# grantjr1842/index-tts

Measured on AMD Instinct MI355X. Metric: synthesised audio seconds per second (IndexTTS-2 infer_v2 hot path), whole job, higher is better.
Workload: dtype f32 (greedy decode + its prefill: exact fp32 MFMA; fp32 accumulate and fp32 activations everywhere) + split-bf16 (fp32 operands as hi+lo bf16, 3 bf16 MFMAs per product) GEMMs, DiT attention and convolutions in s2mel, the latent pass and the vocoder; GPT linear weights STORED as bf16 (rounded once at

## Files before the change

include/idxtts.h:

```cpp
#ifndef IDXTTS_H
#define IDXTTS_H

#include <stddef.h>
#include <stdint.h>

#ifdef __cplusplus
extern "C" {
#endif

typedef struct idxtts_ctx idxtts_ctx;

#define IDXTTS_DTYPE_F32 0
#define IDXTTS_DTYPE_F16 1
#define IDXTTS_DTYPE_BF16 2

int idxtts_version(void);
const char* idxtts_last_error(void);

int idxtts_aa_act_fwd(void* out, const void* in, const float* up_filter, const float* down_filter,
                      const float* log_alpha, const float* log_beta, int B, int C, int T, int dtype,
                      void* stream);

typedef struct idxtts_conv1d idxtts_conv1d;
int idxtts_conv1d_create(const float* weight, const float* bias , int Cout, int Cin, int K,
// ... 39 lines not shown
int idxtts_set_gemm_mode(int mode);
int idxtts_get_gemm_mode(void);
int idxtts_set_acoustic_bf16(int on);
int idxtts_get_acoustic_bf16(void);
int idxtts_set_decode_geometry(int narrow);
int idxtts_get_decode_geometry(void);
int idxtts_set_decode_plane_rows(int min_rows);
int idxtts_get_decode_plane_rows(void);
typedef struct idxtts_gemv_fx_plan {
  int mt, ntw, single, r4, narrow, kw, cps, ksb;
} idxtts_gemv_fx_plan;
int idxtts_gemv_fx_plan_query(int N, int K, int rows, int format, int with_slab, int narrow, idxtts_gemv_fx_plan* out);
int idxtts_gemv_pl_plan_query(int N, int K, int rows, int* ct, int* kparts, int* has_kernel);
int idxtts_s2mel_set_overlap(int on);
int idxtts_s2mel_get_overlap(void);
int idxtts_linear_destroy(idxtts_linear* lin);
int idxtts_release_stream(void* stream);
int idxtts_attention_fwd(const float* q, const float* k, const float* v, float* o, long q_batch_stride, int q_token_stride,
                         long kv_batch_stride, int kv_token_stride, long o_batch_stride, int o_token_stride, int B, int H,
                         int Sq, int Sk, int causal, const int* kstart, const int* kend, float scale, void* stream);
int idxtts_attention_bf16x3_fwd(const float* q, const float* k, const float* v, float* o, long q_batch_stride, int q_token_stride,
                         long kv_batch_stride, int kv_token_stride, long o_batch_stride, int o_token_stride, int B, int H,
                         int Sq, int Sk, int causal, const int* kstart, const int* kend, float scale, void* stream);
int idxtts_attention_bf16_fwd(const float* q, const float* k, const float* v, float* o, long q_batch_stride, int q_token_stride,
                         long kv_batch_stride, int kv_token_stride, long o_batch_stride, int o_token_stride, int B, int H,
                         int Sq, int Sk, int causal, const int* kstart, const int* kend, float scale, void* stream);
int idxtts_attention_relkey_fwd(const float* q, const float* k, const float* v, float* o, long batch_stride, int token_stride,
                                long o_batch_stride, int o_token_stride, int B, int H, int S, const int* kend, float scale,
                                const float* rel_key, int rel_left, int rel_right, int split_bf16, void* stream);
int idxtts_layernorm_fwd(const float* x, float* y, const float* gamma, const float* beta, int M, int d, float eps, void* stream);
// ... 222 lines not shown
```

index-tts_amd/csrc/attention.h:

```cpp
#pragma once
#include "common.h"

namespace idxtts {

struct AttnArgs {
  const float* q = nullptr; const float* k = nullptr; const float* v = nullptr; float* o = nullptr;
  long q_bs = 0, k_bs = 0, v_bs = 0, o_bs = 0;
  int q_ts = 0, k_ts = 0, v_ts = 0, o_ts = 0;
  int B = 0, H = 0, Sq = 0, Sk = 0, head_dim = 64;
  int causal = 0;
  const int* kstart = nullptr;
  const int* kend = nullptr;
  float scale = 0.125f;
  void* o_planes = nullptr;
  int split_bf16 = 0;
  const float* rel_key = nullptr; int rel_left = 0, rel_right = 0;
};

int flash_attn_forward(const AttnArgs& a, hipStream_t stream);

struct AttnPlanesArgs {
  const void* planes = nullptr;
  int Mrows = 0, ncols = 0;
  int q_col = 0, k_col = 0, v_col = 0;
  int T = 0;
// ... 13 lines not shown
```

index-tts_amd/csrc/attention.hip:

```cpp
#include <algorithm>

#include "attention.h"
#include "prof.h"

namespace idxtts {

__device__ __forceinline__ float xor32_max(float v) {
  const auto r = __builtin_amdgcn_permlane32_swap(__float_as_uint(v), __float_as_uint(v), false, false);
  return fmaxf(__uint_as_float(r[0]), __uint_as_float(r[1]));
}
__device__ __forceinline__ float xor32_sum(float v) {
  const auto r = __builtin_amdgcn_permlane32_swap(__float_as_uint(v), __float_as_uint(v), false, false);
  return __uint_as_float(r[0]) + __uint_as_float(r[1]);
}

constexpr int KROW = 68;
constexpr float NEG_BIG = -1e30f;
constexpr int REL_MAX = 96;
constexpr int REL_ROW = 97;
constexpr int REL_LDS = 4 * 32 * REL_ROW * (int)sizeof(float);
constexpr int STAGE_FLOATS = 4 * 32 * 65;

__device__ __forceinline__ int acc_key(int r, int h, int key0 = 0) { return key0 + (r & 3) + 8 * (r >> 2) + 4 * h; }

// ... 8 lines not shown
  w.h = w.lane >> 5; w.j = w.lane & 31;
  w.q0 = qblk * 128 + w.wave * 32;
  w.qi = w.q0 + w.j;
  return w;
}

struct KeyRange {
  int kstart, kend, k_lo, ntiles;
  __device__ __forceinline__ bool sees(int key, int qi, int causal) const { return key >= kstart && key < kend && (!causal || key <= qi); }
};
__device__ __forceinline__ KeyRange visible_keys(const AttnArgs& p, int b, int qblk) {
  KeyRange k;
  k.kstart = p.kstart ? p.kstart[b] : 0;
  k.kend = p.kend ? min(p.kend[b], p.Sk) : p.Sk;
  int k_hi = k.kend;
  if (p.causal) k_hi = min(k_hi, qblk * 128 + 128);
  k.k_lo = k.kstart & ~31;
  k.ntiles = k_hi > k.k_lo ? (k_hi - k.k_lo + 31) >> 5 : 0;
  return k;
}

__device__ __forceinline__ void load_kv(const AttnArgs& p, const float* kb, const float* vb, int key0, int tid, f32x4 (&kr)[2], f32x4 (&vr)[2]) {
#pragma unroll
  for (int l = 0; l < 2; ++l) {
    const int idx = tid + 256 * l;
    const int row = idx >> 4, c4 = idx & 15;
    const int key = key0 + row;
    f32x4 a = {0.f, 0.f, 0.f, 0.f}, c = {0.f, 0.f, 0.f, 0.f};
    if (key < p.Sk) {
      a = *reinterpret_cast<const f32x4*>(kb + (size_t)key * p.k_ts + c4 * 4);
      c = *reinterpret_cast<const f32x4*>(vb + (size_t)key * p.v_ts + c4 * 4);
// ... 118 lines not shown
  extern __shared__ float rel_dyn[];
  float* const tbl_row = rel_dyn + (w.wave * 32 + w.j) * REL_ROW;
  if (p.rel_key)
    build_rel_table(p, w, tbl_row, [&](int row, int c4, f32x4 a) { store_k(0, row, c4, a); }, [&] { return qk_f32(Ks[0], qf, w); });

  if (keys.ntiles > 0) {
    load_kv(p, kb, vb, keys.k_lo, w.tid, kr, vr);
    store_kv(0);
  }
  __syncthreads();
  for (int tile = 0; tile < keys.ntiles; ++tile) {
    const bool has_next = tile + 1 < keys.ntiles;
    const int key0 = keys.k_lo + tile * 32;
    if (has_next) load_kv(p, kb, vb, key0 + 32, w.tid, kr, vr);
    const float* vt = Vs[tile & 1];
    const bool wave_active = !(p.causal && key0 > w.q0 + 31) && w.q0 < p.Sq;
    if (wave_active) {
      f32x16 s = qk_f32(Ks[tile & 1], qf, w);
      if (p.rel_key) add_rel_term(s, tbl_row, key0, w, p.rel_left, p.rel_right);
      float mx = NEG_BIG;
#pragma unroll
      for (int r = 0; r < 16; ++r) {
        s[r] = keys.sees(acc_key(r, w.h, key0), w.qi, p.causal) ? s[r] : NEG_BIG;
        mx = fmaxf(mx, s[r]);
      }
      mx = xor32_max(mx);
      const float m_new = fmaxf(m_run, mx);
      const float alpha = expf(m_run - m_new);
      float psum = 0.0f;
#pragma unroll
      for (int r = 0; r < 16; ++r) {
        const float pv = s[r] <= -1e29f ? 0.0f : expf(s[r] - m_new);
        s[r] = pv;
        psum += pv;
      }
      l_run = l_run * alpha + psum;
      m_run = m_new;
#pragma unroll
// ... 150 lines not shown

  extern __shared__ float rel_dyn[];
  float* const tbl_row = rel_dyn + (w.wave * 32 + w.j) * REL_ROW;
  if (p.rel_key) build_rel_table(p, w, tbl_row, [&](int row, int c4, f32x4 a) { store_k(smem, row, c4, a); }, [&] { return qk(smem); });

  if (keys.ntiles > 0) {
    load_kv(p, kb, vb, keys.k_lo, w.tid, kr, vr);
    store_kv(0);
  }
  __syncthreads();
  for (int tile = 0; tile < keys.ntiles; ++tile) {
    const bool has_next = tile + 1 < keys.ntiles;
    const int key0 = keys.k_lo + tile * 32;
    if (has_next) load_kv(p, kb, vb, key0 + 32, w.tid, kr, vr);
    const char* tb = smem + (tile & 1) * ABUF;
    const bool wave_active = !(p.causal && key0 > w.q0 + 31) && w.q0 < p.Sq;
    if (wave_active) {
      f32x16 s = qk(tb);
      if (p.rel_key) add_rel_term(s, tbl_row, key0, w, p.rel_left, p.rel_right);
      const bool need_mask = key0 < keys.kstart || key0 + 32 > keys.kend || (p.causal && key0 + 31 > w.q0);
      if (need_mask) {
#pragma unroll
        for (int r = 0; r < 16; ++r) s[r] = keys.sees(acc_key(r, w.h, key0), w.qi, p.causal) ? s[r] : NEG_BIG;
      }
      online_softmax_log2<NP == 1>(s, o, m_run, l_run, p.scale * 1.4426950408889634f, need_mask);
      bf16x8 ph[2], pl[2];
      split_p(s, ph, pl);
#pragma unroll
      for (int t2 = 0; t2 < 2; ++t2)
#pragma unroll
        for (int t = 0; t < 2; ++t) {
          const char* va = tb + v_off + 16 * t2 * VB16 + 64 * t;
          typedef __attribute__((address_space(3))) bf16x4 lds_bf16x4;
          const bf16x4 h0 = __builtin_amdgcn_ds_read_tr16_b64_v4bf16((lds_bf16x4*)(va));
          const bf16x4 h1 = __builtin_amdgcn_ds_read_tr16_b64_v4bf16((lds_bf16x4*)(va + 8 * VB16));
          const bf16x8 vh = __builtin_shufflevector(h0, h1, 0, 1, 2, 3, 4, 5, 6, 7);
          bf16x8 vl = vh;
          if constexpr (NP == 3) {
// ... 155 lines not shown
  const double flops = 4.0 * a.B * a.H * (double)a.Sq * a.T * 64;
  const double bytes = 4.0 * a.B * a.H * 64.0 * (2.0 * a.Sq + 2.0 * a.T);
  static const int cat = prof_register("flash_attn_planes_kernel");
  ProfScope prof(cat, stream, flops, bytes);
  IDX_CHECK(a.split_bf16 == 1 || a.split_bf16 == 2, "split_bf16: 1 (three MFMAs per product) or 2 (one)");
  if (a.split_bf16 == 2) hipLaunchKernelGGL(flash_attn_planes_kernel<1>, grid, dim3(256), 0, stream, k);
  else hipLaunchKernelGGL(flash_attn_planes_kernel<3>, grid, dim3(256), 0, stream, k);
  IDX_LAUNCH_CHECK();
  return 0;
}

int flash_attn_forward(const AttnArgs& a, hipStream_t stream) {
  if (a.B == 0 || a.H == 0 || a.Sq == 0) return 0;
  IDX_CHECK(a.q && a.k && a.v && (a.o || (a.o_planes && a.split_bf16)), "null pointer");
  IDX_CHECK(a.head_dim == 64, "head_dim must be 64");
  IDX_CHECK((a.q_ts & 3) == 0 && (a.k_ts & 3) == 0 && (a.v_ts & 3) == 0 && (a.q_bs & 3) == 0 && (a.k_bs & 3) == 0 && (a.v_bs & 3) == 0,
            "q/k/v strides must be multiples of 4 floats");
  dim3 grid(cdiv(a.Sq, 128), a.H, a.B);
  const double flops = 4.0 * a.B * a.H * (double)a.Sq * a.Sk * 64 * (a.causal ? 0.5 : 1.0);
  const double bytes = 4.0 * a.B * a.H * 64.0 * (2.0 * a.Sq + 2.0 * a.Sk);
  static const int cat_x3 = prof_register("flash_attn_bf16x3_kernel"), cat_f32 = prof_register("flash_attn_f32_kernel");
  ProfScope prof(a.split_bf16 ? cat_x3 : cat_f32, stream, flops, bytes);
  size_t dyn = 0;
  if (a.rel_key) {
    IDX_CHECK(a.rel_left >= 0 && a.rel_right >= 0 && a.rel_left + a.rel_right + 1 <= REL_MAX && !a.causal && a.Sq == a.Sk && !a.kstart,
              "relative_key: non-causal self-attention, at most 96 distances");
    IDX_CHECK((reinterpret_cast<uintptr_t>(a.rel_key) & 15) == 0, "rel_key must be 16-byte aligned");
    dyn = REL_LDS;
    static DynLdsLimit lds_limit;
    IDX_CHECK(a.split_bf16 != 2, "relative_key has no single-product form");
// ... 12 lines not shown
```

index-tts_amd/csrc/capi.hip:

```cpp
#include <cstring>
#include <new>

#include "../../include/idxtts.h"
#include "bigvgan.h"
#include "cond.h"
#include "semantic.h"
#include "codec.h"
#include "audio.h"
#include "campplus.h"
#include "conv1d.h"
#include "ctx.h"
#include "fbank.h"
#include "gpt.h"
#include "model_util.h"
#include "s2mel.h"

namespace idxtts {

static thread_local std::string g_last_error;

void set_error(const std::string& msg) { g_last_error = msg; }
int fail(const char* file, int line, const std::string& msg) {
  const char* base = std::strrchr(file, '/');
  g_last_error = std::string(base ? base + 1 : file) + ":" + std::to_string(line) + ": " + msg;
// ... 851 lines not shown
  API_BEGIN
  IDX_CHECK(ct && kparts && has_kernel && N > 0 && K > 0 && rows > 0 && rows <= 64, "N, K > 0, 1..64 rows");
  gemv_pl_plan(N, K, rows, ct, kparts);
  *has_kernel = gemv_pl_can_run(N, K, rows) ? 1 : 0;
  return 0;
  API_END
}

int idxtts_s2mel_set_overlap(int on) {
  set_s2mel_overlap(on);
  return 0;
}

int idxtts_s2mel_get_overlap(void) { return get_s2mel_overlap(); }

}
```

index-tts_amd/csrc/gpt.h:

```cpp
#pragma once
#include <atomic>
#include <functional>
#include <map>
#include <mutex>
#include <vector>

#include "../../include/idxtts.h"
#include "attention.h"
#include "beam.h"
#include "ctx.h"
#include "decode.h"
#include "gemm.h"
#include "gemv16.h"
#include "gemv_pl.h"
#include "norm.h"
#include "prof.h"

namespace idxtts {

struct BeamBuffers {
  float *proc, *beam_scores;
  int *next_tok, *beam_idx, *seq, *hyp_len, *hyp_slot, *hyp_seq, *hyp_n, *done;
  double *hyp_score, *hyp_worst;
  size_t bytes;
// ... 31 lines not shown
  struct GenScope { GPTModel* m; explicit GenScope(GPTModel* mm) : m(mm) { m->generating.fetch_add(1); } ~GenScope() { m->generating.fetch_sub(1); } };
  size_t kv_layer_bytes(int B, int Smax) const { return (size_t)B * cfg.heads * Smax * 64 * (kv_fmt == 2 ? 1 : kv_fmt ? 2 : 4); }
  size_t kv_layer_scales(int B, int Smax) const { return kv_fmt == 2 ? (size_t)B * cfg.heads * Smax : 0; }
  hipStream_t own_stream = nullptr;
  static constexpr int OOB_SLOTS = 64;
  int* oob_flag = nullptr;
  std::atomic<unsigned> oob_next{0};
  ~GPTModel() override {
    for (GraphSlot& g : graph_cache) g.step.drop();
    for (auto& kv : sessions) kv.second.step.drop();
    if (own_stream) (void)hipStreamDestroy(own_stream);
  }

  struct Buffers {
    float *x, *h, *qkv, *att, *ff;
    char *kcache, *vcache; int Smax;
    float *kscale = nullptr, *vscale = nullptr;
    float *xd, *hd, *attd, *ffd;
    float *xrow, *hrow, *attrow, *ffrow, *stats, *pl_slab; unsigned* pl_cnt;
    float *qkvd, *logits, *slab;
    size_t frag_off, frag_bytes;
    unsigned char* seen; int *finished, *cur_tok, *kstart;
    float* attn_part; unsigned* attn_cnt;
    unsigned* ksb_cnt;
    DecodeState* state;
    long long* codes;
    size_t bytes;
    SlotState* slots = nullptr;
    SlotSampling* slot_samp = nullptr;
    idxtts_sampling samp{0, 1.0f, 0, 1.0f, nullptr, 0};
// ... 8 lines not shown
  std::vector<GraphSlot> graph_cache;
  std::mutex graph_mu;
  unsigned long graph_stamp = 0;
  static constexpr size_t GRAPH_CACHE_MAX = 8;

  explicit GPTModel(const idxtts_gpt_config& c);
  bool accepts(const std::string& name) const override;
  int finalize(std::map<std::string, HostTensor>& t, DeviceArena& arena) override;
  int quantize_weights(std::map<std::string, HostTensor>& t, int fmt);
  Buffers carve(void* ws, int B, int S, int max_new, size_t prefill_rows = 0) const;
  size_t workspace_bytes(int B, int S, int max_new) const;
  struct KvScatter {
    const int* slot_ids = nullptr; const int* len = nullptr; int n = 0; int slots = 0;
    int fan = 1;
  };
  int layer_full(int li, const Buffers& w, int B, int S, const int* kstart, bool store_kv, hipStream_t st, const KvScatter* scatter = nullptr);
  int head_logits(const Buffers& w, int B, const float* x, int ldx, bool x_frag, hipStream_t st);
  int head_and_sample(const Buffers& w, int B, const float* x, int ldx, bool x_frag, float penalty, int codes_ld, float* logits_out,
                      hipStream_t st);
  KvDst kv_dst(int li, const Buffers& w, int rows) const;
  DecodeAttnArgs attn_args(int li, const Buffers& w, int B, int pos_hint) const;
  SampleArgs::Embed tail_embed(const Buffers& w, bool pl) const;
  int decode_step(const Buffers& w, int B, float penalty, int codes_ld, float* logits_base, int pos_hint, hipStream_t st);
  int decode_step_pl(const Buffers& w, int B, float penalty, int codes_ld, float* logits_base, int pos_hint, hipStream_t st);
  int capture_step(const Buffers& w, int B, float penalty, int codes_ld, hipStream_t st, StepGraph* g);
  bool use_pl(int B) const;
  bool fused_tail(const Buffers& w) const;
  int call_stream(hipStream_t user, hipStream_t* st);
  int run_generation(const Buffers& w, const float* inputs_embeds, const int* pad_left_host, int B, int fan, int P, int max_new,
                     float penalty, float* logits_out, bool graph, hipGraphExec_t exec, StepGraph* captured, const int* poll, int poll_n,
                     int poll_every, int* steps_done, hipStream_t st);
// ... 38 lines not shown
  int admit_prefill(Session& s, const SessionBuffers& sb, int n, const float* inputs_embeds, int ld_rows, const int* prompt_lens,
                    const int* ids, const int* caps, int fan, const std::function<int()>& params, int* S, hipStream_t st);
  int session_admit(void* ws, int n, const float* inputs_embeds, int ld_rows, const int* prompt_lens, const int* slot_ids,
                    const int* max_new, hipStream_t st, const idxtts_sampling* per_row = nullptr);
  int session_admit_beam(void* ws, int n, const float* inputs_embeds, int ld_rows, const int* prompt_lens, const int* group_ids,
                         const int* max_new, const idxtts_beam* per_request, hipStream_t st);
  int session_read_beam(Session& s, const SessionBuffers& sb, int slot, long long* codes, int* n_codes, hipStream_t st);
  int session_step(void* ws, int n_steps, int use_graph, int* finished_slots, int* n_finished, hipStream_t st);
  int session_read(void* ws, int slot, long long* codes, int* n_codes, hipStream_t st);
  int session_end(void* ws, int n, const int* slot_ids, bool evict, hipStream_t st);
  int session_release(void* ws);
  int embed(float* out, int rows, const int* text_ids, const int* text_pos_idx, const int* mel_ids, const int* mel_pos_idx,
            const float* extra, const int* extra_idx, hipStream_t st);
};

struct BeamHyp { double score; const int* toks; int len; };
int beam_finalize(int nb, double length_penalty, int hyp_n, const double* hyp_score, const int* hyp_len, const int* hyp_slot,
                  const int* hyp_seq, int seq_ld, bool done, const float* bscore, const int* seq, int steps_done, BeamHyp* best);

}
```

index-tts_amd/csrc/gpt.hip:

```cpp
#include <algorithm>
#include <cstdlib>
#include <cstring>

#include "gpt.h"
#include "model_util.h"

namespace idxtts {

GPTModel::GPTModel(const idxtts_gpt_config& c) : cfg(c) {}

bool GPTModel::accepts(const std::string& name) const {
  static const char* prefixes[] = {"gpt.h.", "gpt.ln_f.", "final_norm.", "mel_head.", "mel_embedding.", "text_embedding.",
                                   "mel_pos_embedding.", "text_pos_embedding.", "speed_emb."};
  for (const char* p : prefixes)
    if (name.rfind(p, 0) == 0) return true;
  return false;
}

static int upload_stream(DeviceArena& arena, const float* w, int N, int K, bool kn, int fmt, int kdepth, WeightStream* ws) {
  ws->N = N; ws->K = K; ws->fmt = fmt; ws->kdepth = kdepth;
  std::vector<unsigned char> buf(wstream_elems(N, K, kdepth) * wfmt_bytes(fmt));
  std::vector<float> scale(N, 1.0f);
  if (pack_wstream(buf.data(), w, N, K, kn, fmt, kdepth, scale.data())) IDX_FAIL("decode weights are not representable in the compact format (quantize_weights not applied?)");
  void* d = nullptr;
// ... 120 lines not shown
  if (tensor_from(t, arena, "mel_pos_embedding.emb.weight", {cfg.mel_pos_len, d}, &mel_pos)) return 1;
  if (tensor_from(t, arena, "text_pos_embedding.emb.weight", {cfg.text_pos_len, d}, &text_pos)) return 1;
  return 0;
}

GPTModel::Buffers GPTModel::carve(void* ws, int B, int S, int max_new, size_t prefill_rows) const {
  const int d = cfg.model_dim, V = cfg.number_mel_codes, L = cfg.layers;
  Buffers b;
  Carver c(ws);
  const size_t rows = prefill_rows ? prefill_rows : (size_t)B * S;
  b.x = c.take<float>(rows * d);
  b.h = c.take<float>(rows * d);
  b.qkv = c.take<float>(rows * 3 * d);
  b.att = c.take<float>(rows * d);
  b.ff = c.take<float>(rows * 4 * d);
  b.Smax = max_new > 0 ? ((S + max_new + 3) & ~3) : 0;
  const size_t cache = (size_t)L * kv_layer_bytes(B, b.Smax);
  b.kcache = c.take<char>(cache);
  b.vcache = c.take<char>(cache);
  if (kv_fmt == 2) {
    b.kscale = c.take<float>((size_t)L * kv_layer_scales(B, b.Smax));
    b.vscale = c.take<float>((size_t)L * kv_layer_scales(B, b.Smax));
  }
  b.xd = c.take<float>(frag_image_floats(B, d));
  b.frag_off = c.off - frag_image_floats(B, d) * sizeof(float);
  b.hd = c.take<float>(frag_image_floats(B, d));
  b.attd = c.take<float>(frag_image_floats(B, d));
  b.ffd = c.take<float>(frag_image_floats(B, 4 * d));
  b.pl_cnt = c.take<unsigned>((size_t)cdiv(std::max(V, 4 * d), 16));
  b.frag_bytes = c.off - b.frag_off;
// ... 10 lines not shown
  b.seen = c.take<unsigned char>((size_t)B * V);
  b.finished = c.take<int>(B);
  b.cur_tok = c.take<int>(B);
  b.kstart = c.take<int>(B);
  b.ksb_cnt = c.take<unsigned>((size_t)cdiv(d, 16));
  b.attn_cnt = c.take<unsigned>((size_t)B * cfg.heads);
  b.attn_part = c.take<float>((size_t)B * cfg.heads * 16 * 66);
  b.state = c.take<DecodeState>(1);
  b.codes = c.take<long long>((size_t)B * (max_new > 0 ? max_new : 0));
  b.bytes = (c.off + 255) & ~(size_t)255;
  return b;
}

size_t GPTModel::workspace_bytes(int B, int S, int max_new) const { return carve(nullptr, B, S, max_new).bytes; }

int GPTModel::layer_full(int li, const Buffers& w, int B, int S, const int* kstart, bool store_kv, hipStream_t st, const KvScatter* scatter) {
  const bool exact = store_kv && kv_fmt != 1;
  auto mm = [&](const LinearWeights& lw, const GemmArgs& ga) { return exact ? gemm_tn_forward(lw, ga, st) : gemm_forward(lw, ga, st); };
  const GPTLayer& L = layers[li];
  const int d = cfg.model_dim, M = B * S;
  RowsNormArgs n1;
  n1.x_in = w.x; n1.ld_in = d; n1.y = w.h; n1.ld_y = d; n1.M = M; n1.d = d; n1.mode = NORM_LN; n1.g1 = L.ln1_g; n1.b1 = L.ln1_b;
  if (rows_norm_forward(n1, st)) return 1;
  GemmArgs g;
  g.x = w.h; g.ldx = d; g.y = w.qkv; g.ldy = 3 * d; g.M = M;
  if (mm(L.attn_l, g)) return 1;
  if (store_kv && scatter) {
    if (kv_store_slots(w.qkv, kv_dst(li, w, scatter->slots), scatter->n, cfg.heads, S, w.Smax, d, scatter->slot_ids, scatter->len, st,
                       scatter->fan)) return 1;
  } else if (store_kv) {
    if (kv_store_prefill(w.qkv, kv_dst(li, w, B), B, cfg.heads, S, w.Smax, d, st)) return 1;
  }
  AttnArgs a;
  a.q = w.qkv; a.k = w.qkv + d; a.v = w.qkv + 2 * d; a.o = w.att;
  a.q_bs = a.k_bs = a.v_bs = (long)S * 3 * d; a.o_bs = (long)S * d;
  a.q_ts = a.k_ts = a.v_ts = 3 * d; a.o_ts = d;
  a.B = B; a.H = cfg.heads; a.Sq = S; a.Sk = S; a.causal = 1; a.kstart = kstart; a.scale = 0.125f;
  a.split_bf16 = !exact && get_gemm_mode() == GEMM_BF16X3;
  if (flash_attn_forward(a, st)) return 1;
  GemmArgs p;
  p.x = w.att; p.ldx = d; p.y = w.x; p.ldy = d; p.res = w.x; p.ldr = d; p.M = M;
  if (mm(L.proj_l, p)) return 1;
  RowsNormArgs n2 = n1;
  n2.g1 = L.ln2_g; n2.b1 = L.ln2_b;
  if (rows_norm_forward(n2, st)) return 1;
  GemmArgs f1;
  f1.x = w.h; f1.ldx = d; f1.y = w.ff; f1.ldy = 4 * d; f1.M = M; f1.act = ACT_GELU_NEW;
  if (mm(L.fc_l, f1)) return 1;
  GemmArgs f2;
  f2.x = w.ff; f2.ldx = 4 * d; f2.y = w.x; f2.ldy = d; f2.res = w.x; f2.ldr = d; f2.M = M;
  if (mm(L.fc2_l, f2)) return 1;
  return 0;
}

int GPTModel::head_logits(const Buffers& w, int B, const float* x, int ldx, bool x_frag, hipStream_t st) {
  const int V = cfg.number_mel_codes, d = cfg.model_dim;
  const bool pl = use_pl(B);
  RowsNormArgs n;
  n.x_in = x; n.ld_in = ldx; n.in_frag = x_frag ? 1 : 0; n.M = B; n.d = d;
  if (pl) { n.y = w.hrow; n.ld_y = d; } else { n.y = w.hd; n.ld_y = d; n.y_frag = 1; }
  n.mode = NORM_LN_LN; n.g1 = lnf_g; n.b1 = lnf_b; n.g2 = fn_g; n.b2 = fn_b;
  if (rows_norm_forward(n, st)) return 1;
  if (pl) {
    GemvPLArgs hv;
    hv.x = w.hrow; hv.ldx = d; hv.rows = B; hv.bias = head_b; hv.y = w.logits; hv.ldy = V; hv.slab = w.pl_slab; hv.counters = w.pl_cnt;
    if (gemv_pl_forward(head_p, hv, st)) return 1;
// ... 169 lines not shown
  IDX_HIP(hipMemcpyAsync(w.seen, seen.data(), seen.size(), hipMemcpyHostToDevice, st));
  const DecodeState s0{P, 1, 0, 0};
  IDX_HIP(hipMemcpyAsync(w.state, &s0, sizeof(s0), hipMemcpyHostToDevice, st));
  const std::vector<int> tok(R, cfg.start_mel_token);
  IDX_HIP(hipMemcpyAsync(w.cur_tok, tok.data(), R * sizeof(int), hipMemcpyHostToDevice, st));
  IDX_HIP(hipStreamSynchronize(st));

  for (int j = 0; j < fan; ++j)
    IDX_HIP(hipMemcpy2DAsync(w.x + (size_t)j * S * d, (size_t)fan * S * d * sizeof(float), inputs_embeds, (size_t)P * d * sizeof(float),
                             (size_t)P * d * sizeof(float), B, hipMemcpyDeviceToDevice, st));
  GatherArgs ga;
  ga.out = w.x + (size_t)P * d; ga.ld_out = S * d; ga.d = d;
  ga.table[0] = mel_emb; ga.idx[0] = w.cur_tok;
  ga.table[1] = mel_pos; ga.idx[1] = w.finished;
  if (gather_sum_rows(ga, R, st)) return 1;
  for (int li = 0; li < cfg.layers; ++li)
    if (layer_full(li, w, R, S, w.kstart, true, st)) return 1;
  if (head_and_sample(w, R, w.x + (size_t)(S - 1) * d, S * d, false, penalty, max_new, logits_out, st)) return 1;
  if (!fused_tail(w) && advance_state(w.state, st)) return 1;

  struct Guard {
    StepGraph g;
    ~Guard() { g.drop(); }
  } cap;
  int n_first = 1;
  if (graph && max_new > 2) {
    if (decode_step(w, R, penalty, max_new, nullptr, S + 1, st)) return 1;
    n_first = 2;
    if (!exec) {
      if (capture_step(w, R, penalty, max_new, st, &cap.g)) return 1;
      exec = cap.g.exec;
    }
// ... 227 lines not shown
    if (fan > 1) stage[n + b] = ids[b];
    stage[s.slots + b] = prompt_lens[b] + 1;
    stage[2 * s.slots + b] = caps[b];
  }
  for (int b = 0; b < rows; ++b) stage[3 * s.slots + b] = b < n ? prompt_lens[b] : -1;
  IDX_HIP(hipMemcpyAsync(sb.ids, stage.data(), (fan > 1 ? 2 : 1) * n * sizeof(int), hipMemcpyHostToDevice, st));
  IDX_HIP(hipMemcpyAsync(sb.klen, stage.data() + s.slots, n * sizeof(int), hipMemcpyHostToDevice, st));
  IDX_HIP(hipMemcpyAsync(sb.cap, stage.data() + 2 * s.slots, n * sizeof(int), hipMemcpyHostToDevice, st));
  IDX_HIP(hipMemcpyAsync(sb.plen, stage.data() + 3 * s.slots, rows * sizeof(int), hipMemcpyHostToDevice, st));
  IDX_HIP(hipStreamSynchronize(st));

  if (session_prefill_input(sb.w.x, inputs_embeds, ld_rows, sb.plen, rows, S, cfg.model_dim, mel_emb, mel_pos, cfg.start_mel_token, st))
    return 1;
  KvScatter sc;
  sc.slot_ids = sb.ids; sc.len = sb.klen; sc.n = n; sc.slots = s.slots; sc.fan = fan;
  for (int li = 0; li < cfg.layers; ++li)
    if (layer_full(li, sb.w, rows, S, nullptr, true, st, &sc)) return 1;
  *S_out = S;
  return 0;
}

int GPTModel::session_admit(void* ws, int n, const float* inputs_embeds, int ld_rows, const int* prompt_lens, const int* slot_ids,
                            const int* caps, hipStream_t st, const idxtts_sampling* per_row) {
  Session* sp = find_session(ws);
  IDX_CHECK(sp, "no decode session on this workspace");
  Session& s = *sp;
  IDX_CHECK(s.num_beams == 0, "a beam session admits with _admit_beam (one idxtts_beam per request)");
  IDX_CHECK(!per_row || s.sampled, "per-request sampling needs a session initialised with IDXTTS_SESSION_SAMPLED");
  GenScope gen_scope(this);
  const int d = cfg.model_dim, V = cfg.number_mel_codes;
  const SessionBuffers sb = carve_session(ws, s.slots, s.max_prompt, s.max_new, s.sampled);
  const Buffers& w = sb.w;
// ... 109 lines not shown
int GPTModel::latent(const float* emb, const int* pad_left_host, int B, int S, int mel_start, int M, float* latent_out, void* ws,
                     size_t ws_bytes, hipStream_t st) {
  IDX_CHECK(emb && latent_out, "null pointer");
  IDX_CHECK(B > 0 && S > 0 && M > 0 && mel_start >= 0 && mel_start + M <= S, "shape");
  IDX_CHECK(ws && ws_bytes >= workspace_bytes(B, S, 0), "workspace too small");
  const int d = cfg.model_dim;
  Buffers w = carve(ws, B, S, 0);
  const int* kstart = nullptr;
  if (pad_left_host) {
    for (int b = 0; b < B; ++b) IDX_CHECK(pad_left_host[b] >= 0 && pad_left_host[b] < mel_start, "pad_left out of range");
    IDX_HIP(hipMemcpyAsync(w.kstart, pad_left_host, B * sizeof(int), hipMemcpyHostToDevice, st));
    IDX_HIP(hipStreamSynchronize(st));
    kstart = w.kstart;
  }
  IDX_HIP(hipMemcpyAsync(w.x, emb, (size_t)B * S * d * sizeof(float), hipMemcpyDeviceToDevice, st));
  for (int li = 0; li < cfg.layers; ++li)
    if (layer_full(li, w, B, S, kstart, false, st)) return 1;
  RowsNormArgs n;
  n.x_in = w.x + (size_t)mel_start * d; n.ld_in = d; n.in_rows_per_batch = M; n.in_batch_stride = (long)S * d;
  n.y = latent_out; n.ld_y = d; n.M = B * M; n.d = d; n.mode = NORM_LN_LN;
  n.g1 = lnf_g; n.b1 = lnf_b; n.g2 = fn_g; n.b2 = fn_b;
  return rows_norm_forward(n, st);
}

int GPTModel::embed(float* out, int rows, const int* text_ids, const int* text_pos_idx, const int* mel_ids, const int* mel_pos_idx,
                    const float* extra, const int* extra_idx, hipStream_t st) {
  GatherArgs ga;
  ga.out = out; ga.ld_out = cfg.model_dim; ga.d = cfg.model_dim;
  ga.table[0] = text_emb; ga.idx[0] = text_ids;
  ga.table[1] = text_pos; ga.idx[1] = text_pos_idx;
  ga.table[2] = mel_emb; ga.idx[2] = mel_ids;
  ga.table[3] = mel_pos; ga.idx[3] = mel_pos_idx;
  ga.table[4] = extra; ga.idx[4] = extra_idx;
  ga.table_rows[0] = cfg.number_text_tokens + 1; ga.table_rows[1] = cfg.text_pos_len;
// ... 15 lines not shown
```

index-tts_amd/indextts_amd/_lib.py:

```python
from __future__ import annotations

import ctypes
import os
from ctypes import POINTER, c_char_p, c_float, c_int, c_int64, c_size_t, c_void_p

_HERE = os.path.dirname(os.path.abspath(__file__))
LIB_PATH = os.path.join(_HERE, "libidxtts_hip.so")

SYMBOLS = [
    "idxtts_version", "idxtts_last_error", "idxtts_aa_act_fwd",
    "idxtts_conv1d_create", "idxtts_conv1d_fwd", "idxtts_conv1d_destroy",
    "idxtts_ctx_load_tensor", "idxtts_ctx_finalize", "idxtts_ctx_get_tensor", "idxtts_ctx_destroy",
    "idxtts_fp8_e4m3_decode", "idxtts_fp8_e4m3_encode", "idxtts_kv_fp8_quantize",
    "idxtts_bigvgan_create", "idxtts_bigvgan_workspace_bytes", "idxtts_bigvgan_fwd", "idxtts_bigvgan_fwd_ragged",
    "idxtts_profile_enable", "idxtts_profile_num_kernels", "idxtts_profile_kernel_name", "idxtts_profile_read", "idxtts_profile_event_overhead",
    "idxtts_linear_create", "idxtts_linear_fwd", "idxtts_linear_destroy", "idxtts_release_stream", "idxtts_attention_fwd", "idxtts_attention_bf16x3_fwd", "idxtts_attention_bf16_fwd", "idxtts_attention_relkey_fwd", "idxtts_layernorm_fwd",
    "idxtts_gpt_create", "idxtts_gpt_quantize_weights", "idxtts_gpt_set_kv_format", "idxtts_gpt_get_kv_format", "idxtts_gpt_workspace_bytes", "idxtts_gpt_embed", "idxtts_gpt_generate", "idxtts_gpt_generate_forced", "idxtts_gpt_generate_sampled", "idxtts_gpt_latent",
    "idxtts_gpt_beam_workspace_bytes", "idxtts_gpt_generate_beam",
    "idxtts_gpt_session_workspace_bytes", "idxtts_gpt_session_init", "idxtts_gpt_session_admit", "idxtts_gpt_session_step",
    "idxtts_gpt_session_read", "idxtts_gpt_session_release", "idxtts_gpt_session_workspace_bytes_ex", "idxtts_gpt_session_init_ex",
    "idxtts_gpt_session_admit_sampled", "idxtts_gpt_session_workspace_bytes_beam", "idxtts_gpt_session_init_beam",
    "idxtts_gpt_session_admit_beam", "idxtts_gpt_session_evict", "idxtts_gpt_session_stop",
    "idxtts_s2mel_create", "idxtts_s2mel_cond_workspace_bytes", "idxtts_s2mel_prepare_cond",
    "idxtts_s2mel_cfm_workspace_bytes", "idxtts_s2mel_cfm", "idxtts_set_gemm_mode", "idxtts_get_gemm_mode", "idxtts_set_acoustic_bf16", "idxtts_get_acoustic_bf16", "idxtts_set_decode_geometry", "idxtts_get_decode_geometry", "idxtts_set_decode_plane_rows", "idxtts_get_decode_plane_rows", "idxtts_gemv_fx_plan_query", "idxtts_gemv_pl_plan_query", "idxtts_s2mel_set_overlap", "idxtts_s2mel_get_overlap",
    "idxtts_s2mel_estimator", "idxtts_s2mel_cfm_rows_workspace_bytes", "idxtts_s2mel_cfm_rows", "idxtts_cfm_noise", "idxtts_s2mel_regulate", "idxtts_cond_create", "idxtts_cond_workspace_bytes", "idxtts_cond_forward", "idxtts_cond_forward_rows", "idxtts_emovec_merge",
    "idxtts_gpt_graph_cache_entries", "idxtts_w2vbert_create", "idxtts_w2vbert_workspace_bytes", "idxtts_w2vbert_forward",
    "idxtts_repcodec_create", "idxtts_repcodec_workspace_bytes", "idxtts_repcodec_quantize",
    "idxtts_melspec_create", "idxtts_melspec_frames", "idxtts_melspec_workspace_bytes", "idxtts_melspec_forward",
    "idxtts_fbank_create", "idxtts_fbank_frames", "idxtts_fbank_workspace_bytes", "idxtts_fbank_forward", "idxtts_resample_forward",
    "idxtts_campplus_create", "idxtts_campplus_workspace_bytes", "idxtts_campplus_forward",
    "idxtts_qwen_create", "idxtts_qwen_set_weight_format", "idxtts_qwen_workspace_bytes", "idxtts_qwen_generate",
    "idxtts_qwen_step_graph_launches", "idxtts_qwen_max_batch", "idxtts_qwen_batch_workspace_bytes", "idxtts_qwen_generate_batch",
    "idxtts_qwen_batch_step_graph_launches",
]


class BigVGANConfigC(ctypes.Structure):
    _fields_ = [
        ("num_mels", c_int), ("upsample_initial_channel", c_int), ("num_upsamples", c_int),
# ... 361 lines not shown
    return {n: int(getattr(out, n)) for n, _ in GemvFxPlanC._fields_}


def gemv_pl_plan(N: int, K: int, rows: int) -> dict:
    ct, kp, ok = c_int(), c_int(), c_int()
    check(load().idxtts_gemv_pl_plan_query(int(N), int(K), int(rows), ctypes.byref(ct), ctypes.byref(kp), ctypes.byref(ok)))
    return {"ct": ct.value, "kparts": kp.value, "has_kernel": bool(ok.value)}


def set_s2mel_overlap(on: bool) -> None:
    check(load().idxtts_s2mel_set_overlap(int(bool(on))))


def get_s2mel_overlap() -> bool:
    return bool(load().idxtts_s2mel_get_overlap())
```

Measured before the change: 164.3.

## Use bf16 planes in GPT full-pass layers and trim last layer to mel tail

The GPT full-sequence layer pass (latent computation and non-exact prefills) now keeps the normalized activations, attention output and FFN hidden state as pre-split bf16 planes when all four layer GEMMs support plane inputs. This avoids re-splitting fp32 activations inside each GEMM. For the latent pass, the final layer computes attention queries, projection and FFN only for the mel tail rows, using a new causal query-position offset in flash attention and a row gather. This skips work on prefix rows whose outputs are discarded, at the cost of more complex indexing and a global toggle.

```diff
diff --git a/include/idxtts.h b/include/idxtts.h
--- a/include/idxtts.h
+++ b/include/idxtts.h
@@ -77,6 +77,8 @@
 int idxtts_gemv_pl_plan_query(int N, int K, int rows, int* ct, int* kparts, int* has_kernel);
 int idxtts_s2mel_set_overlap(int on);
 int idxtts_s2mel_get_overlap(void);
+int idxtts_set_gpt_forward_planes(int on);
+int idxtts_get_gpt_forward_planes(void);
 int idxtts_linear_destroy(idxtts_linear* lin);
 int idxtts_release_stream(void* stream);
 int idxtts_attention_fwd(const float* q, const float* k, const float* v, float* o, long q_batch_stride, int q_token_stride,
diff --git a/index-tts_amd/csrc/attention.h b/index-tts_amd/csrc/attention.h
--- a/index-tts_amd/csrc/attention.h
+++ b/index-tts_amd/csrc/attention.h
@@ -9,6 +9,7 @@
   int q_ts = 0, k_ts = 0, v_ts = 0, o_ts = 0;
   int B = 0, H = 0, Sq = 0, Sk = 0, head_dim = 64;
   int causal = 0;
+  int q_pos0 = 0;
   const int* kstart = nullptr;
   const int* kend = nullptr;
   float scale = 0.125f;
diff --git a/index-tts_amd/csrc/attention.hip b/index-tts_amd/csrc/attention.hip
--- a/index-tts_amd/csrc/attention.hip
+++ b/index-tts_amd/csrc/attention.hip
@@ -46,7 +46,7 @@
   k.kstart = p.kstart ? p.kstart[b] : 0;
   k.kend = p.kend ? min(p.kend[b], p.Sk) : p.Sk;
   int k_hi = k.kend;
-  if (p.causal) k_hi = min(k_hi, qblk * 128 + 128);
+  if (p.causal) k_hi = min(k_hi, p.q_pos0 + qblk * 128 + 128);
   k.k_lo = k.kstart & ~31;
   k.ntiles = k_hi > k.k_lo ? (k_hi - k.k_lo + 31) >> 5 : 0;
   return k;
@@ -195,14 +195,14 @@
     const int key0 = keys.k_lo + tile * 32;
     if (has_next) load_kv(p, kb, vb, key0 + 32, w.tid, kr, vr);
     const float* vt = Vs[tile & 1];
-    const bool wave_active = !(p.causal && key0 > w.q0 + 31) && w.q0 < p.Sq;
+    const bool wave_active = !(p.causal && key0 > p.q_pos0 + w.q0 + 31) && w.q0 < p.Sq;
     if (wave_active) {
       f32x16 s = qk_f32(Ks[tile & 1], qf, w);
       if (p.rel_key) add_rel_term(s, tbl_row, key0, w, p.rel_left, p.rel_right);
       float mx = NEG_BIG;
 #pragma unroll
       for (int r = 0; r < 16; ++r) {
-        s[r] = keys.sees(acc_key(r, w.h, key0), w.qi, p.causal) ? s[r] : NEG_BIG;
+        s[r] = keys.sees(acc_key(r, w.h, key0), p.q_pos0 + w.qi, p.causal) ? s[r] : NEG_BIG;
         mx = fmaxf(mx, s[r]);
       }
       mx = xor32_max(mx);
@@ -383,14 +383,14 @@
     const int key0 = keys.k_lo + tile * 32;
     if (has_next) load_kv(p, kb, vb, key0 + 32, w.tid, kr, vr);
     const char* tb = smem + (tile & 1) * ABUF;
-    const bool wave_active = !(p.causal && key0 > w.q0 + 31) && w.q0 < p.Sq;
+    const bool wave_active = !(p.causal && key0 > p.q_pos0 + w.q0 + 31) && w.q0 < p.Sq;
     if (wave_active) {
       f32x16 s = qk(tb);
       if (p.rel_key) add_rel_term(s, tbl_row, key0, w, p.rel_left, p.rel_right);
-      const bool need_mask = key0 < keys.kstart || key0 + 32 > keys.kend || (p.causal && key0 + 31 > w.q0);
+      const bool need_mask = key0 < keys.kstart || key0 + 32 > keys.kend || (p.causal && key0 + 31 > p.q_pos0 + w.q0);
       if (need_mask) {
 #pragma unroll
-        for (int r = 0; r < 16; ++r) s[r] = keys.sees(acc_key(r, w.h, key0), w.qi, p.causal) ? s[r] : NEG_BIG;
+        for (int r = 0; r < 16; ++r) s[r] = keys.sees(acc_key(r, w.h, key0), p.q_pos0 + w.qi, p.causal) ? s[r] : NEG_BIG;
       }
       online_softmax_log2<NP == 1>(s, o, m_run, l_run, p.scale * 1.4426950408889634f, need_mask);
       bf16x8 ph[2], pl[2];
@@ -576,6 +576,7 @@
   if (a.B == 0 || a.H == 0 || a.Sq == 0) return 0;
   IDX_CHECK(a.q && a.k && a.v && (a.o || (a.o_planes && a.split_bf16)), "null pointer");
   IDX_CHECK(a.head_dim == 64, "head_dim must be 64");
+  IDX_CHECK(a.q_pos0 >= 0 && (a.q_pos0 == 0 || (a.causal && a.q_pos0 + a.Sq <= a.Sk)), "q_pos0: causal only, queries inside the key positions");
   IDX_CHECK((a.q_ts & 3) == 0 && (a.k_ts & 3) == 0 && (a.v_ts & 3) == 0 && (a.q_bs & 3) == 0 && (a.k_bs & 3) == 0 && (a.v_bs & 3) == 0,
             "q/k/v strides must be multiples of 4 floats");
   dim3 grid(cdiv(a.Sq, 128), a.H, a.B);
diff --git a/index-tts_amd/csrc/capi.hip b/index-tts_amd/csrc/capi.hip
--- a/index-tts_amd/csrc/capi.hip
+++ b/index-tts_amd/csrc/capi.hip
@@ -889,4 +889,11 @@
 
 int idxtts_s2mel_get_overlap(void) { return get_s2mel_overlap(); }
 
-}
+int idxtts_set_gpt_forward_planes(int on) {
+  set_gpt_forward_planes(on);
+  return 0;
+}
+
+int idxtts_get_gpt_forward_planes(void) { return get_gpt_forward_planes(); }
+
+}
diff --git a/index-tts_amd/csrc/gpt.h b/index-tts_amd/csrc/gpt.h
--- a/index-tts_amd/csrc/gpt.h
+++ b/index-tts_amd/csrc/gpt.h
@@ -69,6 +69,7 @@
 
   struct Buffers {
     float *x, *h, *qkv, *att, *ff;
+    void *h_p, *att_p, *ff_p;
     char *kcache, *vcache; int Smax;
     float *kscale = nullptr, *vscale = nullptr;
     float *xd, *hd, *attd, *ffd;
@@ -107,7 +108,13 @@
     const int* slot_ids = nullptr; const int* len = nullptr; int n = 0; int slots = 0;
     int fan = 1;
   };
-  int layer_full(int li, const Buffers& w, int B, int S, const int* kstart, bool store_kv, hipStream_t st, const KvScatter* scatter = nullptr);
+  struct FullPass { bool store_kv = false, exact = false, planes = false; };
+  FullPass full_pass(int M, bool store_kv) const;
+  int layers_full(const Buffers& w, int B, int S, const int* kstart, bool store_kv, hipStream_t st, const KvScatter* scatter = nullptr,
+                  int q0 = 0);
+  int tail_q0(int B, int S, int q0) const;
+  int layer_full(int li, const Buffers& w, int B, int S, const int* kstart, const FullPass& fp, hipStream_t st, const KvScatter* scatter,
+                 int q0);
   int head_logits(const Buffers& w, int B, const float* x, int ldx, bool x_frag, hipStream_t st);
   int head_and_sample(const Buffers& w, int B, const float* x, int ldx, bool x_frag, float penalty, int codes_ld, float* logits_out,
                       hipStream_t st);
@@ -176,6 +183,9 @@
             const float* extra, const int* extra_idx, hipStream_t st);
 };
 
+void set_gpt_forward_planes(int on);
+int get_gpt_forward_planes();
+
 struct BeamHyp { double score; const int* toks; int len; };
 int beam_finalize(int nb, double length_penalty, int hyp_n, const double* hyp_score, const int* hyp_len, const int* hyp_slot,
                   const int* hyp_seq, int seq_ld, bool done, const float* bscore, const int* seq, int steps_done, BeamHyp* best);
diff --git a/index-tts_amd/csrc/gpt.hip b/index-tts_amd/csrc/gpt.hip
--- a/index-tts_amd/csrc/gpt.hip
+++ b/index-tts_amd/csrc/gpt.hip
@@ -4,6 +4,7 @@
 
 #include "gpt.h"
 #include "model_util.h"
+#include "s2mel_ops.h"
 
 namespace idxtts {
 
@@ -158,6 +159,7 @@
   b.qkv = c.take<float>(rows * 3 * d);
   b.att = c.take<float>(rows * d);
   b.ff = c.take<float>(rows * 4 * d);
+  b.h_p = b.h; b.att_p = b.att; b.ff_p = b.ff;
   b.Smax = max_new > 0 ? ((S + max_new + 3) & ~3) : 0;
   const size_t cache = (size_t)L * kv_layer_bytes(B, b.Smax);
   b.kcache = c.take<char>(cache);
@@ -198,16 +200,19 @@
 
 size_t GPTModel::workspace_bytes(int B, int S, int max_new) const { return carve(nullptr, B, S, max_new).bytes; }
 
-int GPTModel::layer_full(int li, const Buffers& w, int B, int S, const int* kstart, bool store_kv, hipStream_t st, const KvScatter* scatter) {
-  const bool exact = store_kv && kv_fmt != 1;
+int GPTModel::layer_full(int li, const Buffers& w, int B, int S, const int* kstart, const FullPass& fp, hipStream_t st, const KvScatter* scatter,
+                         int q0) {
+  const bool exact = fp.exact, store_kv = fp.store_kv, planes = fp.planes;
   auto mm = [&](const LinearWeights& lw, const GemmArgs& ga) { return exact ? gemm_tn_forward(lw, ga, st) : gemm_forward(lw, ga, st); };
   const GPTLayer& L = layers[li];
   const int d = cfg.model_dim, M = B * S;
   RowsNormArgs n1;
-  n1.x_in = w.x; n1.ld_in = d; n1.y = w.h; n1.ld_y = d; n1.M = M; n1.d = d; n1.mode = NORM_LN; n1.g1 = L.ln1_g; n1.b1 = L.ln1_b;
+  n1.x_in = w.x; n1.ld_in = d; n1.ld_y = d; n1.M = M; n1.d = d; n1.mode = NORM_LN; n1.g1 = L.ln1_g; n1.b1 = L.ln1_b;
+  if (planes) n1.y_planes = w.h_p; else n1.y = w.h;
   if (rows_norm_forward(n1, st)) return 1;
   GemmArgs g;
-  g.x = w.h; g.ldx = d; g.y = w.qkv; g.ldy = 3 * d; g.M = M;
+  g.ldx = d; g.y = w.qkv; g.ldy = 3 * d; g.M = M;
+  if (planes) g.x_planes = w.h_p; else g.x = w.h;
   if (mm(L.attn_l, g)) return 1;
   if (store_kv && scatter) {
     if (kv_store_slots(w.qkv, kv_dst(li, w, scatter->slots), scatter->n, cfg.heads, S, w.Smax, d, scatter->slot_ids, scatter->len, st,
@@ -215,25 +220,61 @@
   } else if (store_kv) {
     if (kv_store_prefill(w.qkv, kv_dst(li, w, B), B, cfg.heads, S, w.Smax, d, st)) return 1;
   }
+  const int Sp = S - q0, Mp = B * Sp;
   AttnArgs a;
-  a.q = w.qkv; a.k = w.qkv + d; a.v = w.qkv + 2 * d; a.o = w.att;
-  a.q_bs = a.k_bs = a.v_bs = (long)S * 3 * d; a.o_bs = (long)S * d;
+  a.q = w.qkv + (size_t)q0 * 3 * d; a.k = w.qkv + d; a.v = w.qkv + 2 * d;
+  if (planes) a.o_planes = w.att_p; else a.o = w.att;
+  a.q_bs = a.k_bs = a.v_bs = (long)S * 3 * d; a.o_bs = (long)Sp * d;
   a.q_ts = a.k_ts = a.v_ts = 3 * d; a.o_ts = d;
-  a.B = B; a.H = cfg.heads; a.Sq = S; a.Sk = S; a.causal = 1; a.kstart = kstart; a.scale = 0.125f;
+  a.B = B; a.H = cfg.heads; a.Sq = Sp; a.Sk = S; a.causal = 1; a.q_pos0 = q0; a.kstart = kstart; a.scale = 0.125f;
   a.split_bf16 = !exact && get_gemm_mode() == GEMM_BF16X3;
   if (flash_attn_forward(a, st)) return 1;
+  float* const xr = q0 > 0 ? w.qkv : w.x;
+  if (q0 > 0 && gather_tail_rows(xr, d, w.x, d, d, B, S, q0, st)) return 1;
   GemmArgs p;
-  p.x = w.att; p.ldx = d; p.y = w.x; p.ldy = d; p.res = w.x; p.ldr = d; p.M = M;
+  p.ldx = d; p.y = xr; p.ldy = d; p.res = xr; p.ldr = d; p.M = Mp;
+  if (planes) p.x_planes = w.att_p; else p.x = w.att;
   if (mm(L.proj_l, p)) return 1;
   RowsNormArgs n2 = n1;
-  n2.g1 = L.ln2_g; n2.b1 = L.ln2_b;
+  n2.x_in = xr; n2.M = Mp; n2.g1 = L.ln2_g; n2.b1 = L.ln2_b;
   if (rows_norm_forward(n2, st)) return 1;
   GemmArgs f1;
-  f1.x = w.h; f1.ldx = d; f1.y = w.ff; f1.ldy = 4 * d; f1.M = M; f1.act = ACT_GELU_NEW;
+  f1.ldx = d; f1.ldy = 4 * d; f1.M = Mp; f1.act = ACT_GELU_NEW;
+  if (planes) { f1.x_planes = w.h_p; f1.y_planes = w.ff_p; } else { f1.x = w.h; f1.y = w.ff; }
   if (mm(L.fc_l, f1)) return 1;
   GemmArgs f2;
-  f2.x = w.ff; f2.ldx = 4 * d; f2.y = w.x; f2.ldy = d; f2.res = w.x; f2.ldr = d; f2.M = M;
+  f2.ldx = 4 * d; f2.y = xr; f2.ldy = d; f2.res = xr; f2.ldr = d; f2.M = Mp;
+  if (planes) f2.x_planes = w.ff_p; else f2.x = w.ff;
   if (mm(L.fc2_l, f2)) return 1;
+  return 0;
+}
+
+static int g_gpt_forward_planes = 1;
+void set_gpt_forward_planes(int on) { g_gpt_forward_planes = on ? 1 : 0; }
+int get_gpt_forward_planes() { return g_gpt_forward_planes; }
+
+GPTModel::FullPass GPTModel::full_pass(int M, bool store_kv) const {
+  FullPass fp;
+  fp.store_kv = store_kv;
+  fp.exact = store_kv && kv_fmt != 1;
+  if (fp.exact || g_gpt_forward_planes == 0) return fp;
+  const GPTLayer& L0 = layers[0];
+  GemmArgs pr;
+  pr.M = M;
+  fp.planes = true;
+  for (const LinearWeights* lw : {&L0.attn_l, &L0.proj_l, &L0.fc_l, &L0.fc2_l}) fp.planes = fp.planes && gemm_uses_planes(*lw, pr);
+  return fp;
+}
+
+int GPTModel::tail_q0(int B, int S, int q0) const {
+  if (q0 <= 0 || q0 >= S) return 0;
+  return full_pass(B * S, false).planes && full_pass(B * (S - q0), false).planes ? q0 : 0;
+}
+
+int GPTModel::layers_full(const Buffers& w, int B, int S, const int* kstart, bool store_kv, hipStream_t st, const KvScatter* scatter, int q0) {
+  const FullPass fp = full_pass(B * S, store_kv);
+  for (int li = 0; li < cfg.layers; ++li)
+    if (layer_full(li, w, B, S, kstart, fp, st, scatter, li + 1 == cfg.layers ? q0 : 0)) return 1;
   return 0;
 }
 
@@ -433,8 +474,7 @@
   ga.table[0] = mel_emb; ga.idx[0] = w.cur_tok;
   ga.table[1] = mel_pos; ga.idx[1] = w.finished;
   if (gather_sum_rows(ga, R, st)) return 1;
-  for (int li = 0; li < cfg.layers; ++li)
-    if (layer_full(li, w, R, S, w.kstart, true, st)) return 1;
+  if (layers_full(w, R, S, w.kstart, true, st)) return 1;
   if (head_and_sample(w, R, w.x + (size_t)(S - 1) * d, S * d, false, penalty, max_new, logits_out, st)) return 1;
   if (!fused_tail(w) && advance_state(w.state, st)) return 1;
 
@@ -692,8 +732,7 @@
     return 1;
   KvScatter sc;
   sc.slot_ids = sb.ids; sc.len = sb.klen; sc.n = n; sc.slots = s.slots; sc.fan = fan;
-  for (int li = 0; li < cfg.layers; ++li)
-    if (layer_full(li, sb.w, rows, S, nullptr, true, st, &sc)) return 1;
+  if (layers_full(sb.w, rows, S, nullptr, true, st, &sc)) return 1;
   *S_out = S;
   return 0;
 }
@@ -833,10 +872,10 @@
     kstart = w.kstart;
   }
   IDX_HIP(hipMemcpyAsync(w.x, emb, (size_t)B * S * d * sizeof(float), hipMemcpyDeviceToDevice, st));
-  for (int li = 0; li < cfg.layers; ++li)
-    if (layer_full(li, w, B, S, kstart, false, st)) return 1;
+  const int q0 = tail_q0(B, S, mel_start);
+  if (layers_full(w, B, S, kstart, false, st, nullptr, q0)) return 1;
   RowsNormArgs n;
-  n.x_in = w.x + (size_t)mel_start * d; n.ld_in = d; n.in_rows_per_batch = M; n.in_batch_stride = (long)S * d;
+  n.x_in = q0 > 0 ? w.qkv : w.x + (size_t)mel_start * d; n.ld_in = d; n.in_rows_per_batch = M; n.in_batch_stride = (long)(S - q0) * d;
   n.y = latent_out; n.ld_y = d; n.M = B * M; n.d = d; n.mode = NORM_LN_LN;
   n.g1 = lnf_g; n.b1 = lnf_b; n.g2 = fn_g; n.b2 = fn_b;
   return rows_norm_forward(n, st);
diff --git a/index-tts_amd/indextts_amd/_lib.py b/index-tts_amd/indextts_amd/_lib.py
--- a/index-tts_amd/indextts_amd/_lib.py
+++ b/index-tts_amd/indextts_amd/_lib.py
@@ -23,6 +23,7 @@
     "idxtts_gpt_session_admit_beam", "idxtts_gpt_session_evict", "idxtts_gpt_session_stop",
     "idxtts_s2mel_create", "idxtts_s2mel_cond_workspace_bytes", "idxtts_s2mel_prepare_cond",
     "idxtts_s2mel_cfm_workspace_bytes", "idxtts_s2mel_cfm", "idxtts_set_gemm_mode", "idxtts_get_gemm_mode", "idxtts_set_acoustic_bf16", "idxtts_get_acoustic_bf16", "idxtts_set_decode_geometry", "idxtts_get_decode_geometry", "idxtts_set_decode_plane_rows", "idxtts_get_decode_plane_rows", "idxtts_gemv_fx_plan_query", "idxtts_gemv_pl_plan_query", "idxtts_s2mel_set_overlap", "idxtts_s2mel_get_overlap",
+    "idxtts_set_gpt_forward_planes", "idxtts_get_gpt_forward_planes",
     "idxtts_s2mel_estimator", "idxtts_s2mel_cfm_rows_workspace_bytes", "idxtts_s2mel_cfm_rows", "idxtts_cfm_noise", "idxtts_s2mel_regulate", "idxtts_cond_create", "idxtts_cond_workspace_bytes", "idxtts_cond_forward", "idxtts_cond_forward_rows", "idxtts_emovec_merge",
     "idxtts_gpt_graph_cache_entries", "idxtts_w2vbert_create", "idxtts_w2vbert_workspace_bytes", "idxtts_w2vbert_forward",
     "idxtts_repcodec_create", "idxtts_repcodec_workspace_bytes", "idxtts_repcodec_quantize",
@@ -414,3 +415,11 @@
 
 def get_s2mel_overlap() -> bool:
     return bool(load().idxtts_s2mel_get_overlap())
+
+
+def set_gpt_forward_planes(on: bool) -> None:
+    check(load().idxtts_set_gpt_forward_planes(int(bool(on))))
+
+
+def get_gpt_forward_planes() -> bool:
+    return bool(load().idxtts_get_gpt_forward_planes())
```

Result: slower. 158.2 (-3.7%).
